# julienperriercornet/turbosqueeze

Measured on AMD Instinct MI355X. Metric: encode+decode GB/s on enwik9-shaped input (round trip of uncompressed bytes), higher is better.
Workload: dtype u8

## Files before the change

turbosqueeze_amd/csrc/tsq_dec_common.cuh:

```cuda
#pragma once

#include <type_traits>

#include "tsq_common.cuh"

namespace tsq {

#ifdef TSQ_STATS
__device__ unsigned long long g_dec_stats[16];
__device__ unsigned long long g_dec_wave[48];
#define TSQD_T0() unsigned long long t0_ = __builtin_amdgcn_s_memtime()
#define TSQD_ACC(slot) do { unsigned long long t1_ = __builtin_amdgcn_s_memtime(); st_[slot] += t1_ - t0_; t0_ = t1_; } while (0)
#define TSQD_CNT(slot, v) st_[slot] += (v)
#else
#define TSQD_T0() do {} while (0)
#define TSQD_ACC(slot) do {} while (0)
#define TSQD_CNT(slot, v) do {} while (0)
#endif

struct SymCfg {
    static constexpr uint32_t T = 1024;
    static constexpr uint32_t S = 6144;
    static constexpr uint32_t SPAD = 160;
    static constexpr uint32_t OUTC = 2 * S;
    static constexpr uint32_t HOP = 16;
    static constexpr uint32_t MAXG = 512;
    static constexpr uint32_t MAXSN = MAXG / HOP + 2;
    static constexpr uint32_t PER = S / T;
    static constexpr uint32_t TERM = S + SPAD;
    static constexpr uint32_t R = 65536 + OUTC + 64;
    static constexpr uint32_t RPAD = 64;
    static constexpr uint32_t SWORDS = (S + SPAD + 16) / 16;
};
static_assert(SymCfg::R % 16 == 0, "ring phase");
static_assert(SymCfg::R == 77888 && SymCfg::R % 64 == 0, "the record scan skews the ring by out_at & 63: the 64-position grid of the bit map falls on the ring's");
static_assert(SymCfg::OUTC == 12 * SymCfg::T, "twelve bytes per lane");
static_assert(SymCfg::S % SymCfg::T == 0 && SymCfg::SWORDS <= SymCfg::T, "lane counts");
static_assert(SymCfg::MAXG <= SymCfg::T / 2 && SymCfg::MAXG % SymCfg::HOP == 0 && SymCfg::MAXG >= SymCfg::S / 13 + 2 * SymCfg::HOP, "group table");
static_assert(4 * SymCfg::MAXG <= 2 * SymCfg::T, "at most two pairs per lane");

__device__ __forceinline__ void pair_lens(uint32_t sb, uint32_t cc, uint32_t ext, uint32_t& slen, uint32_t& olen)
{
    const uint32_t hi = sb >> 4, lo = sb & 15u;
    const uint32_t lit_hi = cc & 2u, lit_lo = cc & 1u;
    const uint32_t o_hi = (!lit_hi && ext && hi < 3u) ? (hi + 2u) << 4 : hi + 1u;
    const uint32_t o_lo = (!lit_lo && ext && lo < 3u) ? (lo + 2u) << 4 : lo + 1u;
    slen = 1u + (lit_hi ? hi + 1u : 2u) + (lit_lo ? lo + 1u : 2u);
    olen = o_hi + o_lo;
}

struct Image {
    uint32_t op, len, at;
    __device__ __forceinline__ uint32_t lead() const { return at & 3u; }
    __device__ __forceinline__ uint32_t a0() const { return at & ~3u; }
};

__device__ __forceinline__ uint4 prefetch_words(const uint8_t* in, uint32_t at, uint32_t av)
{
    using C = SymCfg;
    const uint32_t tid = threadIdx.x;
    const uint32_t lim = av < C::S + C::SPAD ? av : C::S + C::SPAD;
    uint4 w = make_uint4(0, 0, 0, 0);
    if (tid < C::SWORDS && (tid << 4) + 16u <= lim) __builtin_memcpy(&w, in + at + (tid << 4), 16);
    return w;
}
template <class L>
__device__ __forceinline__ void stage_words(uint8_t* lds, const uint8_t* in, uint32_t at, uint32_t av, uint4 pre)
{
    using C = SymCfg;
    const uint32_t tid = threadIdx.x;
    if (tid < C::SWORDS) {
        uint4 w = pre;
        const uint32_t lim = av < C::S + C::SPAD ? av : C::S + C::SPAD, o = tid << 4;
        if (o < lim && o + 16u > lim) {
            uint32_t b[4] = {0, 0, 0, 0};
            for (uint32_t k = 0; o + k < lim; ++k) b[k >> 2] |= (uint32_t)in[at + o + k] << (8u * (k & 3u));
            w = make_uint4(b[0], b[1], b[2], b[3]);
        }
        *reinterpret_cast<uint4*>(lds + L::sbuf + (tid << 4)) = w;
    }
}

template <class L>
__device__ __forceinline__ void parse_groups(uint8_t* lds, uint32_t slim, uint32_t (&x)[SymCfg::PER])
{
    using C = SymCfg;
    const uint32_t tid = threadIdx.x;
    const uint8_t* const sbuf = lds + L::sbuf;
    uint32_t y[C::PER], c[C::PER];
    {
        uint32_t* const pl = reinterpret_cast<uint32_t*>(lds + L::j4);
        constexpr uint32_t NW = (C::S + C::SPAD) / 4u;
#pragma unroll
        for (uint32_t k = 0; k < (NW + C::T - 1u) / C::T; ++k) {
            const uint32_t w = tid + k * C::T;
            if (w < NW) {
                const uint32_t v = reinterpret_cast<const uint32_t*>(sbuf)[w];
                uint32_t q[4];
#pragma unroll
                for (uint32_t b = 0; b < 4; ++b) {
                    const uint32_t hi = (v >> (8u * b + 4u)) & 15u, lo = (v >> (8u * b)) & 15u;
                    q[b] = 0x03040405u + (lo << 8) + (hi << 16) + ((lo + hi) << 24);
                }
                *reinterpret_cast<uint4*>(pl + 4u * w) = make_uint4(q[0], q[1], q[2], q[3]);
            }
        }
    }
    __syncthreads();
    {
        const uint32_t* const pl = reinterpret_cast<const uint32_t*>(lds + L::j4);
#pragma unroll
        for (uint32_t k = 0; k < C::PER; ++k) { const uint32_t o = tid + k * C::T; c[k] = (uint32_t)sbuf[o] << 3; x[k] = o + 1u; }
#pragma unroll
        for (uint32_t pr = 0; pr < 4; ++pr) {
#pragma unroll
            for (uint32_t k = 0; k < C::PER; ++k) y[k] = pl[x[k]];
#pragma unroll
            for (uint32_t k = 0; k < C::PER; ++k) x[k] += __builtin_amdgcn_ubfe(y[k], (c[k] >> (6u - 2u * pr)) & 0x18u, 8u);
        }
    }
    uint8_t* const j1 = lds + L::j1;
#pragma unroll
    for (uint32_t k = 0; k < C::PER; ++k) { const uint32_t o = tid + k * C::T; j1[o] = (uint8_t)(x[k] - o); x[k] = o < slim ? x[k] : C::TERM; }
    __syncthreads();
}

template <class L>
__device__ __forceinline__ void double_pointers(uint8_t* lds, uint32_t slim, uint32_t (&x)[SymCfg::PER])
{
    using C = SymCfg;
    const uint32_t tid = threadIdx.x;
    const uint8_t* const j1 = lds + L::j1;
    uint16_t* const j2 = reinterpret_cast<uint16_t*>(lds + L::j2);
    uint16_t* const j4 = reinterpret_cast<uint16_t*>(lds + L::j4);
    uint16_t* const j8 = reinterpret_cast<uint16_t*>(lds + L::j8);
    uint16_t* const j16 = reinterpret_cast<uint16_t*>(lds + L::j16);
    uint32_t y[C::PER];
#pragma unroll
    for (uint32_t k = 0; k < C::PER; ++k) { const uint32_t a = x[k] < slim ? x[k] : 0u; y[k] = a + j1[a]; }
#pragma unroll
    for (uint32_t k = 0; k < C::PER; ++k) { x[k] = x[k] < slim ? y[k] : C::TERM; j2[tid + k * C::T] = (uint16_t)x[k]; }
    if (tid <= C::SPAD) { j2[C::S + tid] = (uint16_t)C::TERM; j4[C::S + tid] = (uint16_t)C::TERM; j8[C::S + tid] = (uint16_t)C::TERM; j16[C::S + tid] = (uint16_t)C::TERM; }
    __syncthreads();
    const uint16_t* src = j2;
    uint16_t* const dsts[3] = {j4, j8, j16};
#pragma unroll
    for (uint32_t d = 0; d < 3; ++d) {
#pragma unroll
        for (uint32_t k = 0; k < C::PER; ++k) y[k] = src[x[k]];
#pragma unroll
        for (uint32_t k = 0; k < C::PER; ++k) { x[k] = y[k]; dsts[d][tid + k * C::T] = (uint16_t)x[k]; }
        __syncthreads();
        src = dsts[d];
    }
}

template <class L>
__device__ __forceinline__ uint32_t walk_chain(uint8_t* lds, uint32_t first, uint32_t slim)
{
    using C = SymCfg;
    const uint16_t* const j16 = reinterpret_cast<const uint16_t*>(lds + L::j16);
    uint16_t* const sn = reinterpret_cast<uint16_t*>(lds + L::sn);
    uint32_t* const misc = reinterpret_cast<uint32_t*>(lds + L::misc);
    if (threadIdx.x < 64u) {
        uint32_t x = first, k = 0;
        while (x < slim && k < C::MAXSN) {
            const uint32_t x1 = j16[x];
            const uint32_t x2 = j16[x1];
            sn[k++] = (uint16_t)x;
            if (x1 < slim && k < C::MAXSN) { sn[k++] = (uint16_t)x1; x = x2; }
            else x = x1;
        }
        if (threadIdx.x == 0) { misc[0] = k; if (k >= C::MAXSN && x < slim) misc[4] = kErrStream; }
    }
    __syncthreads();
    return misc[0];
}

template <class L>
__device__ __forceinline__ void group_lanes(uint8_t* lds, uint32_t nsn, uint32_t slim, uint32_t op, uint32_t size, uint32_t ext)
{
    using C = SymCfg;
    const uint32_t tid = threadIdx.x, lane = tid & 63u, wid = tid >> 6;
    const uint8_t* const sbuf = lds + L::sbuf;
    const uint8_t* const j1 = lds + L::j1;
    const uint16_t* const j2 = reinterpret_cast<const uint16_t*>(lds + L::j2);
    const uint16_t* const j4 = reinterpret_cast<const uint16_t*>(lds + L::j4);
    const uint16_t* const j8 = reinterpret_cast<const uint16_t*>(lds + L::j8);
    const uint16_t* const sn = reinterpret_cast<const uint16_t*>(lds + L::sn);
    uint16_t* const gstart = reinterpret_cast<uint16_t*>(lds + L::gstart);
    uint16_t* const glen = reinterpret_cast<uint16_t*>(lds + L::glen);
    uint32_t* const gout = reinterpret_cast<uint32_t*>(lds + L::gout);
    uint32_t* const pairs = reinterpret_cast<uint32_t*>(lds + L::pairs);
    uint32_t* const wsum = reinterpret_cast<uint32_t*>(lds + L::wsum);
    uint32_t* const misc = reinterpret_cast<uint32_t*>(lds + L::misc);
    uint32_t x = C::TERM;
    if (tid < nsn * C::HOP) {
        x = sn[tid >> 4];
        if (tid & 8u) x = j8[x];
        if (tid & 4u) x = j4[x];
        if (tid & 2u) x = j2[x];
        if (tid & 1u) x = x < slim ? (uint32_t)(x + j1[x]) : C::TERM;
    }
    uint32_t v = 0;
    if (x < slim) {
        gstart[tid] = (uint16_t)x;
        const uint32_t c = sbuf[x];
        uint32_t p = x + 1u, pw[4];
#pragma unroll
        for (uint32_t pr = 0; pr < 4; ++pr) {
            const uint32_t cc = (c >> (6u - 2u * pr)) & 3u;
            pw[pr] = p | (v << 13) | (cc << 30);
            uint32_t sl, ol;
            pair_lens(sbuf[p], cc, ext, sl, ol);
            p += sl;
            v += ol;
        }
        *reinterpret_cast<uint4*>(pairs + tid * 4u) = make_uint4(pw[0], pw[1], pw[2], pw[3]);
        glen[tid] = (uint16_t)v;
        if (p >= slim) { misc[1] = tid + 1u; misc[5] = p; }
    }
    const uint32_t incl = wave_scan_add(v);
    if (lane == 63) wsum[wid] = incl;
    __syncthreads();
    const uint32_t totals = wave_scan_add(lane < C::T / 64u ? wsum[lane] : 0u);
    const uint32_t before = wid ? (uint32_t)__builtin_amdgcn_readlane((int)totals, (int)wid - 1) : 0u;
    const uint32_t excl = before + incl - v;
    if (x < slim) {
        gout[tid] = op + excl;
        if (excl + 512u + 16u > C::OUTC) atomicMin(&misc[2], tid);
        if (op + excl + v >= size) atomicMin(&misc[3], tid);
    }
}

struct ChunkEnd {
    uint32_t ng;
    uint32_t next_at;
    uint32_t next_op;
    bool last;
    bool cut;
};
template <class L>
__device__ __forceinline__ ChunkEnd chunk_end(const uint8_t* lds, uint32_t op, uint32_t size)
{
    const uint16_t* const gstart = reinterpret_cast<const uint16_t*>(lds + L::gstart);
    const uint16_t* const glen = reinterpret_cast<const uint16_t*>(lds + L::glen);
    const uint32_t* const gout = reinterpret_cast<const uint32_t*>(lds + L::gout);
    const uint32_t* const misc = reinterpret_cast<const uint32_t*>(lds + L::misc);
    const uint32_t ng = misc[1], cut = misc[2], fin = misc[3];
    if (fin != 0xFFFFFFFFu && fin < cut) return {fin + 1u, 0u, size, true, false};
    if (cut != 0xFFFFFFFFu) return {cut, gstart[cut], gout[cut], false, true};
    return {ng, misc[5], ng ? gout[ng - 1] + glen[ng - 1] : op, false, false};
}

template <class L>
__device__ __forceinline__ void clear_records(uint8_t* lds)
{
    uint32_t* const recw = reinterpret_cast<uint32_t*>(lds + L::recw);
    for (uint32_t w = threadIdx.x; w < (SymCfg::OUTC + 16) / 4; w += SymCfg::T) *reinterpret_cast<uint4*>(recw + 4u * w) = make_uint4(0, 0, 0, 0);
}
template <class L, class PairAt>
__device__ __forceinline__ void drop_records(uint8_t* lds, uint32_t ng, const Image& im, uint32_t size, uint32_t avail, uint32_t ext,
                                             PairAt pair_at)
{
    using C = SymCfg;
    const uint32_t tid = threadIdx.x;
    const uint8_t* const sbuf = lds + L::sbuf;
    uint32_t* const recw = reinterpret_cast<uint32_t*>(lds + L::recw);
    const uint32_t op = im.op, lead = im.lead(), a0 = im.a0();
    if (tid == 0 && lead) recw[0] = 0x40000000u | (L::ring + a0);
    uint32_t bad = 0;
#pragma unroll
    for (uint32_t rep = 0; rep < 2; ++rep) {
        const uint32_t gi = tid + rep * C::T;
        if (gi >= ng * 4u) break;
        const uint2 pg = pair_at(rep, gi);
        const uint32_t pw = pg.x;
        uint32_t p = pw & 0x1FFFu, j = pg.y + ((pw >> 13) & 0x3FFFu);
        const uint32_t origin = j;
        uint32_t sb = 0;
        if (j < size) { if (p >= avail) bad = 1; sb = sbuf[p]; p++; }
#pragma unroll
        for (uint32_t sidx = 0; sidx < 2; ++sidx) {
            if (j < size && !bad) {
                const uint32_t nib = sidx == 0 ? sb >> 4 : sb & 15u;
                const uint32_t lit = (pw >> (31u - sidx)) & 1u;
                const uint32_t room = size - j;
                const uint32_t ij = j - op + lead;
                if (lit) {
                    const uint32_t len = nib + 1u, take = len < room ? len : room;
                    if (p + take > avail) bad = 1;
                    else recw[ij] = 0x40000000u | ((L::sbuf + p - ij) & 0xFFFFFFu);
                    p += len; j += take;
                } else {
                    if (p + 2u > avail) bad = 1;
                    const uint32_t off = (uint32_t)sbuf[p] | ((uint32_t)sbuf[p + 1] << 8);
                    p += 2;
                    const uint32_t len = ext ? nibble_span(nib) : nib + 1u;
                    const uint32_t take = len < room ? len : room;
                    if (off > origin || take > off) bad = 1;
                    if (!bad) {
                        const uint32_t a = origin - off;
                        const uint32_t n_hist = a >= op ? 0u : (op - a < take ? op - a : take);
                        if (n_hist) {
                            uint32_t x0 = a0 + C::R - ((op - a) - lead);
                            x0 -= x0 >= C::R ? C::R : 0u;
                            recw[ij] = 0x40000000u | ((L::ring + x0 - ij) & 0xFFFFFFu);
                            if (x0 + n_hist > C::R) { const uint32_t n1 = C::R - x0; recw[ij + n1] = 0x40000000u | ((L::ring - (ij + n1)) & 0xFFFFFFu); }
                        }
                        if (n_hist < take) recw[ij + n_hist] = 0xC0000000u | ((a - j) & 0xFFFFFFu);
                    }
                    j += take;
                }
            }
        }
    }
    if (bad) reinterpret_cast<uint32_t*>(lds + L::misc)[4] = kErrStream;
}

typedef __attribute__((address_space(3))) uint16_t lds_u16;

template <class L>
__device__ __forceinline__ uint32_t fetch_bytes(uint8_t* lds, const Image& im)
{
    const uint32_t tid = threadIdx.x, lane = tid & 63u, wid = tid >> 6;
    const uint32_t* const recw = reinterpret_cast<const uint32_t*>(lds + L::recw);
    uint32_t* const wsum = reinterpret_cast<uint32_t*>(lds + L::wsum);
    lds_u16* const wl = (lds_u16*)(lds + L::plist) + 768u * wid;
    const uint32_t own = 12u * tid;
    uint32_t r[12];
    {
        const uint4 q0 = *reinterpret_cast<const uint4*>(recw + own), q1 = *reinterpret_cast<const uint4*>(recw + own + 4u),
                    q2 = *reinterpret_cast<const uint4*>(recw + own + 8u);
        r[0] = q0.x; r[1] = q0.y; r[2] = q0.z; r[3] = q0.w; r[4] = q1.x; r[5] = q1.y; r[6] = q1.z; r[7] = q1.w; r[8] = q2.x; r[9] = q2.y; r[10] = q2.z; r[11] = q2.w;
#pragma unroll
        for (uint32_t k = 1; k < 12; ++k) r[k] = r[k] ? r[k] : r[k - 1];
        const uint32_t upto = wave_scan_last(r[11]);
        uint32_t carry = (uint32_t)__builtin_amdgcn_update_dpp(0, (int)upto, 0x138, 0xF, 0xF, false);
        if (lane == 63) wsum[wid] = upto;
        __syncthreads();
        {
            const uint32_t ws = lane < 16u ? wsum[lane] : 0u;
            const uint64_t m = __ballot(ws != 0u && lane < wid);
            const uint32_t prev = m ? (uint32_t)__builtin_amdgcn_readlane((int)ws, 63 - __builtin_clzll(m)) : 0u;
            carry = carry ? carry : prev;
        }
#pragma unroll
        for (uint32_t k = 0; k < 12; ++k) r[k] = r[k] ? r[k] : carry;
    }
    uint32_t pend = 0;
    if (own < im.lead() + im.len) {
        uint32_t v[12], by[12];
#pragma unroll
        for (uint32_t k = 0; k < 12; ++k) {
            v[k] = own + k + (uint32_t)((int32_t)(r[k] << 8) >> 8);
// ... 212 lines not shown
```

turbosqueeze_amd/csrc/tsq_dec_sym.cuh:

```cuda
#pragma once

#include "tsq_common.cuh"
#include "tsq_dec_common.cuh"

namespace tsq {

struct SymLds {
    static constexpr uint32_t sbuf = 0;
    static constexpr uint32_t j1 = sbuf + 16 * SymCfg::SWORDS;
    static constexpr uint32_t JN = (SymCfg::S + SymCfg::SPAD + 8u) & ~7u;
    static constexpr uint32_t j2 = j1 + SymCfg::S;
    static constexpr uint32_t j4 = j2 + 2 * JN;
    static constexpr uint32_t j8 = j4 + 2 * JN;
    static constexpr uint32_t j16 = j8 + 2 * JN;
    static constexpr uint32_t recw = j1;
    static constexpr uint32_t ent = j1;
    static constexpr uint32_t plist = ent + 2 * (SymCfg::OUTC + 16);
    static constexpr uint32_t gstart = j16 + 2 * JN;
    static constexpr uint32_t glen = gstart + 2 * SymCfg::MAXG;
    static constexpr uint32_t gout = glen + 2 * SymCfg::MAXG;
    static constexpr uint32_t pairs = gout + 4 * SymCfg::MAXG;
    static constexpr uint32_t sn = pairs + 16 * SymCfg::MAXG;
    static constexpr uint32_t wsum = (sn + 2 * ((SymCfg::MAXSN + 7) & ~7u) + 15) & ~15u;
    static constexpr uint32_t misc = wsum + 64;
    static constexpr uint32_t ring = (misc + 64 + 15) & ~15u;
    static constexpr uint32_t total = ring + SymCfg::R + SymCfg::RPAD;
    static_assert(recw % 16 == 0 && recw + 4 * (SymCfg::OUTC + 16) <= gstart && plist % 16 == 0 && plist + 2 * SymCfg::OUTC <= gstart,
                  "records, byte entries and waiting lists fit the dead doubling tables");
};
static_assert(SymLds::total <= 160 * 1024, "LDS budget");

struct RangeItem {
    uint32_t block, lo, hi, pad;
    uint64_t out_at;
};

struct BlockGroup {
    uint32_t block, first, count, hi;
};

enum DecMode : int { kDecWhole, kDecWindow, kDecGroup, kDecMark, kDecFind };

struct GroupCursor {
    uint32_t cur = 0, cur_lo = 0;
    uint32_t held = 0xFFFFFFFFu;
    RangeItem it = {0u, 0u, 0u, 0u, 0ull};
};

template <class L>
__device__ __forceinline__ void flush_group(const uint8_t* lds, uint8_t* out, const Image& im, const RangeItem* items, uint32_t count, GroupCursor& gc,
                                            uint32_t first_tid, uint32_t n_threads)
{
    using C = SymCfg;
    const uint32_t tid = threadIdx.x;
    if (im.len == 0 || tid < first_tid || gc.cur >= count || gc.cur_lo >= im.op + im.len) return;
    uint32_t& cur = gc.cur;
    const uint8_t* const ring = lds + L::ring;
    const uint32_t lane = tid & 63u, w = (tid - first_tid) >> 6, nw = n_threads >> 6;
    const uint32_t im_end = im.op + im.len;
    uint32_t pass0 = 0;
    bool leading = true;
    for (uint32_t base = cur & ~63u; base < count; base += 64u) {
        const uint32_t k = base + lane;
        RangeItem it = {0u, 0xFFFFFFFFu, 0u, 0u, 0ull};
        if (base == gc.held) it = gc.it;
        else if (k < count) it = items[k];
        const bool in_run = it.lo < im_end;
        if (leading) {
            gc.held = base; gc.it = it;
            const uint64_t done = __ballot(k < count && it.hi <= im.op);
            const uint32_t n = ~done == 0ull ? 64u : (uint32_t)__builtin_ctzll(~done);
            cur = base + n;
            leading = n == 64u;
            if (!leading) gc.cur_lo = (uint32_t)__builtin_amdgcn_readlane((int)it.lo, (int)n);
        }
        const uint32_t a = it.lo > im.op ? it.lo : im.op, b = it.hi < im_end ? it.hi : im_end;
        const bool live = in_run && a < b;
        const uint32_t len = live ? b - a : 0u;
        const uint64_t addr = (uint64_t)(uintptr_t)out + it.out_at + (a - it.lo);
        const uint32_t nwords = live ? (((uint32_t)addr & 15u) + len + 15u) >> 4 : 0u;
        uint32_t ra = im.at + (a - im.op); ra -= ra >= C::R ? C::R : 0u;
        uint32_t incl = nwords;
#pragma unroll
        for (uint32_t d = 1; d < 64u; d <<= 1) {
            const uint32_t up = __shfl_up(incl, d);
            if (lane >= d) incl += up;
        }
        const uint32_t total = (uint32_t)__builtin_amdgcn_readlane((int)incl, 63);
        const uint32_t passes = (total + 63u) >> 6;
        const uint32_t packed = len | (ra << 14);
        for (uint32_t j = (w + nw - pass0 % nw) % nw; j < passes; j += nw) {
            const uint32_t q = (j << 6) + lane;
            uint32_t t = 0;
#pragma unroll
            for (uint32_t step = 32u; step != 0u; step >>= 1) {
                const uint32_t v = __shfl(incl, (int)(t + step - 1u));
                t += v <= q ? step : 0u;
            }
            const bool act = q < total;
            const int src = (int)(t & 63u);
            const uint32_t excl_s = __shfl(incl - nwords, src), alo = __shfl((uint32_t)addr, src), ahi = __shfl((uint32_t)(addr >> 32), src),
                           pk = __shfl(packed, src);
            if (act) {
                const uint32_t kk = q - excl_s, slen = pk & 0x3FFFu, sra = pk >> 14, s = alo & 15u;
                uint8_t* const word = reinterpret_cast<uint8_t*>((uintptr_t)((((uint64_t)ahi << 32) | alo) & ~15ull)) + ((size_t)kk << 4);
                const int32_t i0 = (int32_t)(kk << 4) - (int32_t)s;
                const uint32_t e0 = kk == 0u ? s : 0u;
                const uint32_t left = (uint32_t)((int32_t)slen - i0), e1 = left < 16u ? left : 16u;
                int32_t r = (int32_t)sra + i0;
                r += r < 0 ? (int32_t)C::R : 0; r -= r >= (int32_t)C::R ? (int32_t)C::R : 0;
                const uint32_t r0 = (uint32_t)r & ~15u;
                uint32_t r1 = r0 + 16u; r1 -= r1 >= C::R ? C::R : 0u;
                const uint4 x = *reinterpret_cast<const uint4*>(ring + r0), y = *reinterpret_cast<const uint4*>(ring + r1);
                const uint32_t v8[8] = {x.x, x.y, x.z, x.w, y.x, y.y, y.z, y.w};
                const uint32_t dsh = ((uint32_t)r >> 2) & 3u, bsh = ((uint32_t)r & 3u) << 3;
                uint32_t u[5], o[4];
#pragma unroll
                for (uint32_t i = 0; i < 5u; ++i) u[i] = dsh == 0u ? v8[i] : dsh == 1u ? v8[i + 1] : dsh == 2u ? v8[i + 2] : v8[i + 3];
#pragma unroll
                for (uint32_t i = 0; i < 4u; ++i) o[i] = (uint32_t)((((uint64_t)u[i + 1] << 32) | u[i]) >> bsh);
                if (e0 == 0u && e1 == 16u) {
                    *reinterpret_cast<uint4*>(word) = make_uint4(o[0], o[1], o[2], o[3]);
                } else {
#pragma unroll
                    for (uint32_t i = 0; i < 4u; ++i) {
                        if (e0 <= 4u * i && 4u * i + 4u <= e1) {
                            *reinterpret_cast<uint32_t*>(word + 4u * i) = o[i];
                        } else {
#pragma unroll
                            for (uint32_t c = 0; c < 4u; ++c)
                                if (4u * i + c >= e0 && 4u * i + c < e1) word[4u * i + c] = (uint8_t)(o[i] >> (8u * c));
                        }
                    }
                }
            }
        }
        pass0 += passes;
        if (__ballot(!in_run) != 0ull) break;
    }
}

template <DecMode kMode>
__device__ __forceinline__ void sym_decode_block(const uint8_t* container, const FrameInfo* frames, uint32_t n_frames, const RangeItem* items,
                                                 uint8_t* outbuf, int32_t* status, const BlockGroup* groups = nullptr, uint32_t n_items = 0u,
                                                 [[maybe_unused]] uint32_t delim = 0u, [[maybe_unused]] uint64_t map_words = 0ull,
                                                 [[maybe_unused]] FindNeedle needle = {0ull, 0ull, 0u}, [[maybe_unused]] uint8_t* edges = nullptr)
{
    constexpr bool kWindow = kMode == kDecWindow, kGroup = kMode == kDecGroup, kMark = kMode == kDecMark, kFind = kMode == kDecFind;
    using C = SymCfg;
    using L = SymLds;
    extern __shared__ __attribute__((aligned(16))) uint8_t lds[];
    const uint32_t* const gout = reinterpret_cast<const uint32_t*>(lds + L::gout);
    const uint32_t* const pairs = reinterpret_cast<const uint32_t*>(lds + L::pairs);
    uint32_t* const misc = reinterpret_cast<uint32_t*>(lds + L::misc);

    const uint32_t tid = threadIdx.x;
    if (tid == 0) misc[11] = (uint32_t)*status;
    __syncthreads();
    if (misc[11] != 0u) return;
    uint32_t blk = blockIdx.x, lo = 0, hi = 0;
    uint64_t out_at = 0;
    if constexpr (kWindow) {
        const RangeItem it = items[blockIdx.x];
        if (it.block >= n_frames) {
            if (tid == 0) atomicMax(status, kErrStream);
            return;
        }
        blk = it.block; lo = it.lo; hi = it.hi; out_at = it.out_at;
    }
    [[maybe_unused]] const RangeItem* gitems = nullptr;
    [[maybe_unused]] uint32_t gcount = 0;
    [[maybe_unused]] GroupCursor gcur;
    if constexpr (kGroup) {
        const BlockGroup g = groups[blockIdx.x];
        if (g.block >= n_frames || g.count == 0u || g.first > n_items || g.count > n_items - g.first) {
            if (tid == 0) atomicMax(status, kErrStream);
            return;
        }
        blk = g.block; hi = g.hi; gitems = items + g.first; gcount = g.count;
    }
    const FrameInfo f = frames[blk];
    if (f.stream_len < 3u || f.stream_len > kSlotSize || f.out_len > kBlockSize || ((kWindow || kGroup) && (lo >= hi || hi > f.out_len))) {
        if (tid == 0) atomicMax(status, kErrStream);
        return;
    }
    const uint8_t* const in = container + f.stream_at;
    uint8_t* const out = kGroup || kMark || kFind ? outbuf : outbuf + (kWindow ? out_at : f.out_at);
    const uint32_t in_len = f.stream_len, size = f.out_len, ext = f.ext;
    const uint32_t oskew = kMark || kFind ? (uint32_t)(f.out_at & 63u) : kGroup ? 0u : (uint32_t)(((uintptr_t)out - lo) & 15u);

#ifdef TSQ_STATS
    const uint32_t lane = tid & 63u, wid = tid >> 6;
    unsigned long long st_[16] = {0};
    unsigned long long wj_[3] = {0, 0, 0};
#endif
    TSQD_T0();
    if (tid == 0) { misc[4] = 0; misc[9] = 0; misc[10] = 0; }
    uint32_t sp = 3, op = 0;
    uint32_t ring_op = oskew;
    Image prev = {0, 0, 0};
    uint4 pre = prefetch_words(in, sp, in_len - sp);
    bool staged_ahead = false;
    __syncthreads();

    while (op < size) {
        const uint32_t avail = in_len - sp;
        const uint32_t slim = avail < C::S ? avail : C::S;
        if (!staged_ahead) stage_words<L>(lds, in, sp, avail, pre);
        if (tid == 0) { misc[0] = 0; misc[1] = 0; misc[2] = 0xFFFFFFFFu; misc[3] = 0xFFFFFFFFu; misc[5] = 0; }
        __syncthreads();
        TSQD_ACC(0); TSQD_CNT(12, 1);

        uint32_t x[C::PER];
        parse_groups<L>(lds, slim, x);
        TSQD_ACC(1);
        double_pointers<L>(lds, slim, x);
        TSQD_ACC(2);
        const uint32_t nsn = walk_chain<L>(lds, 0u, slim);
        TSQD_ACC(3);

        if (tid >= C::T / 2) {
            if constexpr (kFind) flush_find<L>(lds, reinterpret_cast<uint32_t*>(out), map_words, f.out_at, blk, prev, needle, size, edges, C::T / 2, C::T / 2);
            else if constexpr (kMark) flush_mark<L>(lds, reinterpret_cast<uint32_t*>(out), map_words, f.out_at, blk, prev, delim, C::T / 2, C::T / 2);
            else if constexpr (kGroup) flush_group<L>(lds, out, prev, gitems, gcount, gcur, C::T / 2, C::T / 2);
            else if constexpr (kWindow) flush_window<L>(lds, out, prev, lo, hi, C::T / 2, C::T / 2);
            else flush_image<L>(lds, out, prev, C::T / 2, C::T / 2);
        }
        group_lanes<L>(lds, nsn, slim, op, size, ext);
        clear_records<L>(lds);
        __syncthreads();
        const ChunkEnd e = chunk_end<L>(lds, op, size);
        const uint32_t next_sp = sp + e.next_at;
        if (misc[4] != 0 || e.ng == 0 || (!e.last && next_sp >= in_len)) {
            if (tid == 0) atomicMax(status, kErrStream);
            return;
        }
        const Image im = {op, e.next_op - op, ring_op};
        const bool more = !e.last && !((kWindow || kGroup) && e.next_op >= hi);
        if (more) pre = prefetch_words(in, next_sp, in_len - next_sp);
        TSQD_ACC(4);

        drop_records<L>(lds, e.ng, im, size, avail, ext,
                        [&](uint32_t, uint32_t gi) { return make_uint2(pairs[gi], gout[gi >> 2]); });
        __syncthreads();
        if (misc[4] != 0) { if (tid == 0) atomicMax(status, (int32_t)misc[4]); return; }
        TSQD_ACC(5);
        const uint32_t n_wait = fetch_bytes<L>(lds, im);
        __syncthreads();
        TSQD_ACC(6);
        if (more) { stage_words<L>(lds, in, next_sp, in_len - next_sp, pre); staged_ahead = true; }
#ifdef TSQ_STATS
        const unsigned long long wj0_ = __builtin_amdgcn_s_memtime();
#endif
        [[maybe_unused]] const uint32_t iters = jump_pointers<L>(lds, n_wait);
#ifdef TSQ_STATS
        if (lane == 0) { atomicMax(&misc[9], iters); atomicAdd(&misc[10], n_wait); }
        if (lane == 0 && blockIdx.x == 0) { wj_[0] += __builtin_amdgcn_s_memtime() - wj0_; wj_[1] += n_wait; wj_[2] += iters; }
#endif
        __syncthreads();
        write_ring<L>(lds, im);
        TSQD_ACC(7);
#ifdef TSQ_STATS
        if (tid == 0) { st_[14] += misc[9]; st_[11] += misc[10]; misc[9] = 0; misc[10] = 0; }
#endif

        prev = im;
        ring_op += im.len; ring_op -= ring_op >= C::R ? C::R : 0u;
        op = e.next_op;
        sp = next_sp;
        TSQD_ACC(8);
        if (!more) break;
    }
    if constexpr (kGroup) { if (tid == C::T / 2) misc[12] = gcur.cur; }
    __syncthreads();
    if constexpr (kGroup) { if (tid < C::T / 2) gcur.cur = misc[12]; }
    if constexpr (kFind) flush_find<L>(lds, reinterpret_cast<uint32_t*>(out), map_words, f.out_at, blk, prev, needle, size, edges, 0, C::T);
    else if constexpr (kMark) flush_mark<L>(lds, reinterpret_cast<uint32_t*>(out), map_words, f.out_at, blk, prev, delim, 0, C::T);
    else if constexpr (kGroup) flush_group<L>(lds, out, prev, gitems, gcount, gcur, 0, C::T);
    else if constexpr (kWindow) flush_window<L>(lds, out, prev, lo, hi, 0, C::T);
    else flush_image<L>(lds, out, prev, 0, C::T);
#ifdef TSQ_STATS
    if (blockIdx.x == 0 && tid == 0) for (int q = 0; q < 16; ++q) g_dec_stats[q] = st_[q];
    if (blockIdx.x == 0 && lane == 0) for (int q = 0; q < 3; ++q) g_dec_wave[wid * 3 + q] = wj_[q];
#endif
}

__global__ __launch_bounds__(1024) void dec_sym_kernel(const uint8_t* __restrict__ container, const FrameInfo* __restrict__ frames,
                                                       uint8_t* __restrict__ outbuf, int32_t* __restrict__ status)
{
    sym_decode_block<kDecWhole>(container, frames, 0u, nullptr, outbuf, status);
}

__global__ __launch_bounds__(1024) void dec_item_kernel(const uint8_t* __restrict__ container, const FrameInfo* __restrict__ frames,
                                                        const uint32_t* __restrict__ owner, uint8_t* __restrict__ outbuf,
                                                        int32_t* __restrict__ item_status, const uint32_t* __restrict__ live_blocks)
{
    if (live_blocks && blockIdx.x >= *live_blocks) return;
    sym_decode_block<kDecWhole>(container, frames, 0u, nullptr, outbuf, item_status + owner[blockIdx.x]);
}

__global__ __launch_bounds__(1024) void dec_range_kernel(const uint8_t* __restrict__ container, const FrameInfo* __restrict__ frames, uint32_t n_frames,
                                                         const RangeItem* __restrict__ items, uint8_t* __restrict__ outbuf, int32_t* __restrict__ status)
{
    sym_decode_block<kDecWindow>(container, frames, n_frames, items, outbuf, status);
}

__global__ __launch_bounds__(1024) void dec_group_kernel(const uint8_t* __restrict__ container, const FrameInfo* __restrict__ frames, uint32_t n_frames,
                                                         const RangeItem* __restrict__ items, uint32_t n_items, const BlockGroup* __restrict__ groups,
                                                         uint8_t* __restrict__ outbuf, int32_t* __restrict__ status)
{
    sym_decode_block<kDecGroup>(container, frames, n_frames, items, outbuf, status, groups, n_items);
}

__global__ __launch_bounds__(1024) void dec_mark_kernel(const uint8_t* __restrict__ container, const FrameInfo* __restrict__ frames,
                                                        const int32_t* __restrict__ verdict, uint32_t delim, uint64_t* __restrict__ map,
                                                        uint64_t map_words, int32_t* __restrict__ status)
{
    if (verdict && *verdict != 0) return;
    sym_decode_block<kDecMark>(container, frames, 0u, nullptr, reinterpret_cast<uint8_t*>(map), status, nullptr, 0u, delim, map_words);
}

__global__ __launch_bounds__(1024) void dec_find_kernel(const uint8_t* __restrict__ container, const FrameInfo* __restrict__ frames,
                                                        const int32_t* __restrict__ verdict, uint32_t n0, uint32_t n1, uint32_t n2, uint32_t n3,
                                                        uint32_t m, uint64_t* __restrict__ map, uint64_t map_words, uint8_t* __restrict__ edges,
                                                        int32_t* __restrict__ status)
{
    if (verdict && *verdict != 0) return;
    const FindNeedle needle = {((uint64_t)n1 << 32) | n0, ((uint64_t)n3 << 32) | n2, m};
    sym_decode_block<kDecFind>(container, frames, 0u, nullptr, reinterpret_cast<uint8_t*>(map), status, nullptr, 0u, 0u, map_words, needle, edges);
}

}
```

turbosqueeze_amd/csrc/tsq_experiment.h:

```cpp
#pragma once

#if defined(TSQ_X_NOHAZ) || defined(TSQ_X_NOCOMMITWAIT) || defined(TSQ_X_NOPATCH) || defined(TSQ_X_FAKE_TABLE) || defined(TSQ_X_FAKE_CAND) || \
    defined(TSQ_X_FREE_QUERY)
#define TSQ_TIMING_ONLY_BUILD 1
#ifndef TSQ_EXPERIMENT
#error "a timing-only switch (TSQ_X_*: wrong streams on purpose) needs -DTSQ_EXPERIMENT; the product library is never built with one (tools/xbuild.sh)"
#endif
#else
#define TSQ_TIMING_ONLY_BUILD 0
#endif

#if defined(TSQ_STATS) || defined(TSQ_SPINS) || defined(TSQ_TRACEONLY) || defined(TSQ_REGION) || defined(TSQ_JITTER) || defined(TSQ_X_DELAY_STAGE)
#define TSQ_INSTRUMENTED_BUILD 1
#else
#define TSQ_INSTRUMENTED_BUILD 0
#endif
```

turbosqueeze_amd/csrc/tsq_runtime.hip:

```cpp
#include "tsq_internal.h"

#include "tsq_batch.cuh"
#include "tsq_common.cuh"
#include "tsq_container.cuh"
#include "tsq_format.h"
#include "tsq_serial.cuh"
#include "tsq_split.cuh"
#include "tsq_index.cuh"
#include "tsq_index_packed.cuh"
#include "tsq_join.cuh"
#include "tsq_cut.cuh"
#include "tsq_launch.cuh"
#include "tsq_gather.cuh"
#include "tsq_gather_sort.h"
#include "tsq_rows.cuh"
#include "tsq_records.cuh"
#include "tsq_find.cuh"

#include <algorithm>
#include <cstdarg>
#include <cstdio>
#include <cstring>
#include <memory>
#include <new>

using namespace tsq;

#define TSQ_HIP(ctx, call)                                                                       \
    do {                                                                                         \
        hipError_t e_ = (call);                                                                  \
        if (e_ != hipSuccess) {                                                                  \
            (ctx)->set_error("%s failed: %s", #call, hipGetErrorString(e_));                     \
            return TSQA_ERR_HIP;                                                                 \
        }                                                                                        \
    } while (0)

void tsqa_ctx::set_error(const char* fmt, ...)
{
    va_list ap;
    va_start(ap, fmt);
    vsnprintf(err, sizeof(err), fmt, ap);
    va_end(ap);
}

static hipStream_t stream_of(const tsqa_ctx* c, void* hip_stream) { return hip_stream ? static_cast<hipStream_t>(hip_stream) : c->stream; }

extern "C" size_t tsqa_block_count(size_t n) { return (n + kBlockSize - 1) / kBlockSize; }

extern "C" size_t tsqa_container_bound(size_t n) { return 16 + tsqa_block_count(n) * (size_t)(3 + kSlotSize); }

#define TSQ_STR2(x) #x
#define TSQ_STR(x) TSQ_STR2(x)
#if !defined(TSQ_LM) || !defined(TSQ_LF) || !defined(TSQ_RECORDS)
#error "tsqa_build_info stringifies TSQ_LM, TSQ_LF and TSQ_RECORDS: tsq_enc_stage.cuh (through tsq_launch.cuh) goes above it"
#endif
extern "C" const char* tsqa_build_info(void)
{
    return "arch=gfx950 timing_only=" TSQ_STR(TSQ_TIMING_ONLY_BUILD) " instrumented=" TSQ_STR(TSQ_INSTRUMENTED_BUILD)
#ifdef TSQ_AB_VARIANTS
           " ab_variants=1"
#else
           " ab_variants=0"
#endif
           " lm=" TSQ_STR(TSQ_LM) " lf=" TSQ_STR(TSQ_LF) " records=" TSQ_STR(TSQ_RECORDS) " [switches:"
#ifdef TSQ_X_NOHAZ
           " TSQ_X_NOHAZ"
#endif
#ifdef TSQ_X_NOCOMMITWAIT
           " TSQ_X_NOCOMMITWAIT"
#endif
#ifdef TSQ_X_NOPATCH
           " TSQ_X_NOPATCH"
#endif
#ifdef TSQ_X_FAKE_TABLE
           " TSQ_X_FAKE_TABLE"
#endif
#ifdef TSQ_X_FAKE_CAND
           " TSQ_X_FAKE_CAND"
#endif
#ifdef TSQ_X_FREE_QUERY
           " TSQ_X_FREE_QUERY"
#endif
#ifdef TSQ_X_DELAY_STAGE
           " TSQ_X_DELAY_STAGE"
#endif
#ifdef TSQ_STATS
           " TSQ_STATS"
#endif
#ifdef TSQ_SPINS
           " TSQ_SPINS"
#endif
#ifdef TSQ_TRACEONLY
           " TSQ_TRACEONLY"
#endif
#ifdef TSQ_JITTER
           " TSQ_JITTER"
#endif
#if !TSQ_TIMING_ONLY_BUILD && !TSQ_INSTRUMENTED_BUILD
           " none"
#endif
           "]";
}

extern "C" int tsqa_create(int device, tsqa_ctx** out)
{
    if (!out) return TSQA_ERR_ARG;
    *out = nullptr;
    int count = 0;
    if (hipGetDeviceCount(&count) != hipSuccess || count <= 0) return TSQA_ERR_NO_DEVICE;
    if (device < 0) { if (hipGetDevice(&device) != hipSuccess) return TSQA_ERR_NO_DEVICE; }
    if (device >= count) return TSQA_ERR_ARG;
    hipDeviceProp_t prop;
    if (hipGetDeviceProperties(&prop, device) != hipSuccess) return TSQA_ERR_NO_DEVICE;
    if (strncmp(prop.gcnArchName, "gfx950", 6) != 0) {
        fprintf(stderr, "turbosqueeze_amd: device %d is %s; this library carries gfx950 code only\n", device, prop.gcnArchName);
        return TSQA_ERR_NO_DEVICE;
    }
    tsqa_ctx* c = new (std::nothrow) tsqa_ctx();
    if (!c) return TSQA_ERR_ARG;
    c->device = device;
    c->n_cus = prop.multiProcessorCount;
    if (const char* e = getenv("TSQ_AMD_DECODE_WAIT_LIMIT")) { const long v = atol(e); if (v > 0) c->decode_wait_limit = (uint32_t)v; }
    if (hipSetDevice(device) != hipSuccess || hipStreamCreateWithFlags(&c->stream, hipStreamNonBlocking) != hipSuccess) {
        delete c;
        return TSQA_ERR_HIP;
    }
    if (!c->d_size.grow(c, 1) || !c->d_status.grow(c, 1)) {
        tsqa_destroy(c);
        return TSQA_ERR_HIP;
    }
    *out = c;
    return TSQA_OK;
}

extern "C" void tsqa_destroy(tsqa_ctx* c)
{
    if (!c) return;
    (void)hipSetDevice(c->device);
    if (c->stream) { (void)hipStreamSynchronize(c->stream); (void)hipStreamDestroy(c->stream); }
    for (hipEvent_t e : c->prof_pool) if (e) (void)hipEventDestroy(e);
    if (c->host_frames_copied) (void)hipEventDestroy(c->host_frames_copied);
    c->range_up.destroy(); c->batch_up.destroy();
    delete c;
}

extern "C" const char* tsqa_last_error(const tsqa_ctx* c) { return c ? c->err : "null context"; }
extern "C" int tsqa_device_id(const tsqa_ctx* c) { return c ? c->device : -1; }
extern "C" void tsqa_set_kernel_variant(tsqa_ctx* c, int ev, int dv) { if (c) { c->enc_variant = ev; c->dec_variant = dv; } }
extern "C" void tsqa_set_decode_wait_limit(tsqa_ctx* c, uint32_t polls) { if (c) c->decode_wait_limit = polls ? polls : 1u; }

int tsqa_ctx::reserve(size_t n_blocks, bool want_tables, bool want_slots, bool all_streams, hipStream_t s)
{
    (void)hipSetDevice(device);
    const size_t nb = n_blocks, n_at = nb ? nb + 1 : 0;
    const size_t n_slots = want_slots && nb ? nb * (size_t)kSlotSize + 256 : 0, n_tables = want_tables ? nb * (size_t)kHashEntries : 0;
    const bool descriptors = sizes.needs(nb) || frame_at.needs(n_at) || frames.needs(nb) || block_owner.needs(nb);
    if (!descriptors && !slots.needs(n_slots) && !tables.needs(n_tables)) return TSQA_OK;
    if (all_streams) (void)hipDeviceSynchronize(); else wait_for(s);
    if (descriptors) forget_sharded();
    return sizes.grow(this, nb) && frame_at.grow(this, n_at) && frames.grow(this, nb) && block_owner.grow(this, nb) &&
           slots.grow(this, n_slots) && tables.grow(this, n_tables) ? TSQA_OK : TSQA_ERR_HIP;
}

int tsqa_ctx::reserve_duo(size_t n_blocks, hipStream_t s)
{
    (void)hipSetDevice(device);
    const size_t n_ring = n_blocks * (size_t)DuoCfg::SLOTS * DuoCfg::REC_WORDS, n_flags = n_blocks * (size_t)DuoCfg::FLAG_STRIDE;
    if (!duo_ring.needs(n_ring) && !duo_flags.needs(n_flags)) return TSQA_OK;
    wait_for(s);
    return duo_ring.grow(this, n_ring) && duo_flags.grow(this, n_flags) ? TSQA_OK : TSQA_ERR_HIP;
}

static size_t doubled(size_t from, size_t n)
{
    if (n == 0) return 0;
    while (from < n) from *= 2;
    return from;
}

int tsqa_ctx::reserve_host_frames(size_t n)
{
    (void)hipSetDevice(device);
    if (host_frames_pending) { (void)hipEventSynchronize(host_frames_copied); host_frames_pending = false; }
    if (!host_frames_copied) TSQ_HIP(this, hipEventCreateWithFlags(&host_frames_copied, hipEventDisableTiming));
    if (host_frames.needs(n)) TSQ_HIP(this, host_frames.grow(doubled(64, n)));
    host_frame_src.resize(host_frames.cap);
    return TSQA_OK;
}

int tsqa_uploads::acquire(tsqa_ctx* c, size_t bytes, Slot* slot)
{
    (void)hipSetDevice(c->device);
    const int k = next_;
    next_ ^= 1;
    if (pending_[k]) { (void)hipEventSynchronize(done_[k]); pending_[k] = false; }
    if (!done_[k]) TSQ_HIP(c, hipEventCreateWithFlags(&done_[k], hipEventDisableTiming));
    if (dev_[k].needs(bytes)) {
        const size_t want = doubled(4096, bytes);
        host_[k].reset(); dev_[k].reset();
        TSQ_HIP(c, host_[k].grow(want));
        if (!dev_[k].grow(c, want)) return TSQA_ERR_HIP;
    }
    *slot = Slot{this, k};
    return TSQA_OK;
}

void tsqa_uploads::destroy()
{
    for (int k = 0; k < 2; ++k)
        if (done_[k]) (void)hipEventDestroy(done_[k]);
}

int tsqa_ctx::reserve_batch(size_t n_items)
{
    (void)hipSetDevice(device);
    const size_t want = doubled(256, n_items), one = want ? 1 : 0;
    if (!batch_at.needs(want) && !batch_sizes.needs(want) && !batch_offsets.needs(want + one) && !batch_heads.needs(want * kHeaderSize) &&
        !batch_status.needs(want) && !batch_items.needs(want) && !batch_live.needs(one)) return TSQA_OK;
    (void)hipDeviceSynchronize();
    return batch_at.grow(this, want) && batch_sizes.grow(this, want) && batch_offsets.grow(this, want + one) &&
           batch_heads.grow(this, want * kHeaderSize) && batch_status.grow(this, want) && batch_items.grow(this, want) &&
           batch_live.grow(this, one) ? TSQA_OK : TSQA_ERR_HIP;
}

int tsqa_ctx::reserve_tables(size_t n_blocks, size_t n_launches, bool want_items)
{
    (void)hipSetDevice(device);
    const size_t blocks = doubled(256, n_blocks), launches = doubled(16, n_launches), owners = want_items ? blocks : 0;
    if (!table_blocks.needs(blocks) && !table_launch_item.needs(launches) && !table_block_item.needs(owners)) return TSQA_OK;
    (void)hipDeviceSynchronize();
    return table_blocks.grow(this, blocks) && table_launch_item.grow(this, launches) && table_block_item.grow(this, owners) ? TSQA_OK : TSQA_ERR_HIP;
}

int tsqa_ctx::reserve_join(size_t n_items)
// ... 2750 lines not shown
```

Measured before the change: 22.77.

## Build pointer-jumping with two doubling tables instead of four in symbol decoder

The decoder's pointer doubling now stores only a 4-hop and a 16-hop table. It reaches the 4-hop table by walking the 1-hop byte table three times in registers, and the 16-hop table by chaining the 4-hop table three times. This cuts two LDS table writes and two block barriers. The group lane seeding then uses up to three 4-hop plus three 1-hop lookups instead of one lookup per power of two, trading more dependent LDS reads for fewer syncs and less LDS. The group tables move down over the freed space, and a timing-only experimental switch is added that skips parsing by replaying cached tables.

```diff
diff --git a/turbosqueeze_amd/csrc/tsq_dec_common.cuh b/turbosqueeze_amd/csrc/tsq_dec_common.cuh
--- a/turbosqueeze_amd/csrc/tsq_dec_common.cuh
+++ b/turbosqueeze_amd/csrc/tsq_dec_common.cuh
@@ -131,28 +131,30 @@
     using C = SymCfg;
     const uint32_t tid = threadIdx.x;
     const uint8_t* const j1 = lds + L::j1;
-    uint16_t* const j2 = reinterpret_cast<uint16_t*>(lds + L::j2);
     uint16_t* const j4 = reinterpret_cast<uint16_t*>(lds + L::j4);
-    uint16_t* const j8 = reinterpret_cast<uint16_t*>(lds + L::j8);
     uint16_t* const j16 = reinterpret_cast<uint16_t*>(lds + L::j16);
     uint32_t y[C::PER];
 #pragma unroll
-    for (uint32_t k = 0; k < C::PER; ++k) { const uint32_t a = x[k] < slim ? x[k] : 0u; y[k] = a + j1[a]; }
-#pragma unroll
-    for (uint32_t k = 0; k < C::PER; ++k) { x[k] = x[k] < slim ? y[k] : C::TERM; j2[tid + k * C::T] = (uint16_t)x[k]; }
-    if (tid <= C::SPAD) { j2[C::S + tid] = (uint16_t)C::TERM; j4[C::S + tid] = (uint16_t)C::TERM; j8[C::S + tid] = (uint16_t)C::TERM; j16[C::S + tid] = (uint16_t)C::TERM; }
+    for (uint32_t h = 0; h < 3; ++h) {
+#pragma unroll
+        for (uint32_t k = 0; k < C::PER; ++k) { const uint32_t a = x[k] < slim ? x[k] : 0u; y[k] = a + j1[a]; }
+#pragma unroll
+        for (uint32_t k = 0; k < C::PER; ++k) x[k] = x[k] < slim ? y[k] : C::TERM;
+    }
+#pragma unroll
+    for (uint32_t k = 0; k < C::PER; ++k) j4[tid + k * C::T] = (uint16_t)x[k];
+    if (tid <= C::SPAD) { j4[C::S + tid] = (uint16_t)C::TERM; j16[C::S + tid] = (uint16_t)C::TERM; }
     __syncthreads();
-    const uint16_t* src = j2;
-    uint16_t* const dsts[3] = {j4, j8, j16};
-#pragma unroll
-    for (uint32_t d = 0; d < 3; ++d) {
-#pragma unroll
-        for (uint32_t k = 0; k < C::PER; ++k) y[k] = src[x[k]];
-#pragma unroll
-        for (uint32_t k = 0; k < C::PER; ++k) { x[k] = y[k]; dsts[d][tid + k * C::T] = (uint16_t)x[k]; }
-        __syncthreads();
-        src = dsts[d];
-    }
+#pragma unroll
+    for (uint32_t h = 0; h < 3; ++h) {
+#pragma unroll
+        for (uint32_t k = 0; k < C::PER; ++k) y[k] = j4[x[k]];
+#pragma unroll
+        for (uint32_t k = 0; k < C::PER; ++k) x[k] = y[k];
+    }
+#pragma unroll
+    for (uint32_t k = 0; k < C::PER; ++k) j16[tid + k * C::T] = (uint16_t)x[k];
+    __syncthreads();
 }
 
 template <class L>
@@ -184,9 +186,7 @@
     const uint32_t tid = threadIdx.x, lane = tid & 63u, wid = tid >> 6;
     const uint8_t* const sbuf = lds + L::sbuf;
     const uint8_t* const j1 = lds + L::j1;
-    const uint16_t* const j2 = reinterpret_cast<const uint16_t*>(lds + L::j2);
     const uint16_t* const j4 = reinterpret_cast<const uint16_t*>(lds + L::j4);
-    const uint16_t* const j8 = reinterpret_cast<const uint16_t*>(lds + L::j8);
     const uint16_t* const sn = reinterpret_cast<const uint16_t*>(lds + L::sn);
     uint16_t* const gstart = reinterpret_cast<uint16_t*>(lds + L::gstart);
     uint16_t* const glen = reinterpret_cast<uint16_t*>(lds + L::glen);
@@ -197,10 +197,11 @@
     uint32_t x = C::TERM;
     if (tid < nsn * C::HOP) {
         x = sn[tid >> 4];
-        if (tid & 8u) x = j8[x];
-        if (tid & 4u) x = j4[x];
-        if (tid & 2u) x = j2[x];
-        if (tid & 1u) x = x < slim ? (uint32_t)(x + j1[x]) : C::TERM;
+        const uint32_t h4 = (tid >> 2) & 3u, h1 = tid & 3u;
+#pragma unroll
+        for (uint32_t h = 0; h < 3; ++h) if (h < h4) x = j4[x];
+#pragma unroll
+        for (uint32_t h = 0; h < 3; ++h) if (h < h1) x = x < slim ? (uint32_t)(x + j1[x]) : C::TERM;
     }
     uint32_t v = 0;
     if (x < slim) {
diff --git a/turbosqueeze_amd/csrc/tsq_dec_sym.cuh b/turbosqueeze_amd/csrc/tsq_dec_sym.cuh
--- a/turbosqueeze_amd/csrc/tsq_dec_sym.cuh
+++ b/turbosqueeze_amd/csrc/tsq_dec_sym.cuh
@@ -9,14 +9,12 @@
     static constexpr uint32_t sbuf = 0;
     static constexpr uint32_t j1 = sbuf + 16 * SymCfg::SWORDS;
     static constexpr uint32_t JN = (SymCfg::S + SymCfg::SPAD + 8u) & ~7u;
-    static constexpr uint32_t j2 = j1 + SymCfg::S;
-    static constexpr uint32_t j4 = j2 + 2 * JN;
-    static constexpr uint32_t j8 = j4 + 2 * JN;
-    static constexpr uint32_t j16 = j8 + 2 * JN;
+    static constexpr uint32_t j4 = j1 + SymCfg::S;
+    static constexpr uint32_t j16 = j4 + 2 * JN;
     static constexpr uint32_t recw = j1;
     static constexpr uint32_t ent = j1;
     static constexpr uint32_t plist = ent + 2 * (SymCfg::OUTC + 16);
-    static constexpr uint32_t gstart = j16 + 2 * JN;
+    static constexpr uint32_t gstart = recw + 4 * (SymCfg::OUTC + 16);
     static constexpr uint32_t glen = gstart + 2 * SymCfg::MAXG;
     static constexpr uint32_t gout = glen + 2 * SymCfg::MAXG;
     static constexpr uint32_t pairs = gout + 4 * SymCfg::MAXG;
@@ -26,9 +24,14 @@
     static constexpr uint32_t ring = (misc + 64 + 15) & ~15u;
     static constexpr uint32_t total = ring + SymCfg::R + SymCfg::RPAD;
     static_assert(recw % 16 == 0 && recw + 4 * (SymCfg::OUTC + 16) <= gstart && plist % 16 == 0 && plist + 2 * SymCfg::OUTC <= gstart,
-                  "records, byte entries and waiting lists fit the dead doubling tables");
+                  "records, byte entries and waiting lists lie over the dead doubling tables, below the group tables");
+    static_assert(j4 % 16 == 0 && j4 + 4 * (SymCfg::S + SymCfg::SPAD) <= gstart && j16 + 2 * JN <= gstart, "P1's pair lengths and both doubling tables");
 };
 static_assert(SymLds::total <= 160 * 1024, "LDS budget");
+#ifdef TSQ_X_DEC_FREEPARSE
+struct SymLdsX { static constexpr uint32_t sbuf = SymLds::pairs; };
+static_assert(SymLdsX::sbuf % 16 == 0 && 16 * SymCfg::SWORDS <= 16 * SymCfg::MAXG, "the stream fits the pair words");
+#endif
 
 struct RangeItem {
     uint32_t block, lo, hi, pad;
@@ -201,21 +204,40 @@
     Image prev = {0, 0, 0};
     uint4 pre = prefetch_words(in, sp, in_len - sp);
     bool staged_ahead = false;
+#ifdef TSQ_X_DEC_FREEPARSE
+    constexpr uint32_t kXWarm = 8;
+    constexpr uint32_t kXTab = (L::j16 + 2 * L::JN - L::j1) / 16;
+    static_assert((L::j16 + 2 * L::JN - L::j1) % 16 == 0 && kXTab <= 2 * C::T, "two words per lane");
+    uint4 xtab[2] = {make_uint4(0, 0, 0, 0), make_uint4(0, 0, 0, 0)};
+    uint32_t xsp = sp;
+    uint32_t xn = 0;
+#endif
     __syncthreads();
 
     while (op < size) {
         const uint32_t avail = in_len - sp;
         const uint32_t slim = avail < C::S ? avail : C::S;
         if (!staged_ahead) stage_words<L>(lds, in, sp, avail, pre);
+#ifdef TSQ_X_DEC_FREEPARSE
+        if (xn > kXWarm) for (uint32_t q = 0; q < 2; ++q) if (tid + q * C::T < kXTab) *reinterpret_cast<uint4*>(lds + L::j1 + 16u * (tid + q * C::T)) = xtab[q];
+#endif
         if (tid == 0) { misc[0] = 0; misc[1] = 0; misc[2] = 0xFFFFFFFFu; misc[3] = 0xFFFFFFFFu; misc[5] = 0; }
         __syncthreads();
         TSQD_ACC(0); TSQD_CNT(12, 1);
 
         uint32_t x[C::PER];
+#ifdef TSQ_X_DEC_FREEPARSE
+        if (xn <= kXWarm) {
+            parse_groups<L>(lds, slim, x);
+            double_pointers<L>(lds, slim, x);
+            if (xn == kXWarm) for (uint32_t q = 0; q < 2; ++q) if (tid + q * C::T < kXTab) xtab[q] = *reinterpret_cast<const uint4*>(lds + L::j1 + 16u * (tid + q * C::T));
+        }
+#else
         parse_groups<L>(lds, slim, x);
         TSQD_ACC(1);
         double_pointers<L>(lds, slim, x);
         TSQD_ACC(2);
+#endif
         const uint32_t nsn = walk_chain<L>(lds, 0u, slim);
         TSQD_ACC(3);
 
@@ -237,7 +259,12 @@
         }
         const Image im = {op, e.next_op - op, ring_op};
         const bool more = !e.last && !((kWindow || kGroup) && e.next_op >= hi);
+#ifdef TSQ_X_DEC_FREEPARSE
+        xsp = xsp + e.next_at < in_len ? xsp + e.next_at : 3u;
+        if (more) pre = prefetch_words(in, xsp, in_len - xsp);
+#else
         if (more) pre = prefetch_words(in, next_sp, in_len - next_sp);
+#endif
         TSQD_ACC(4);
 
         drop_records<L>(lds, e.ng, im, size, avail, ext,
@@ -248,7 +275,11 @@
         const uint32_t n_wait = fetch_bytes<L>(lds, im);
         __syncthreads();
         TSQD_ACC(6);
+#ifdef TSQ_X_DEC_FREEPARSE
+        if (more) { if (xn < kXWarm) stage_words<L>(lds, in, xsp, in_len - xsp, pre); else stage_words<SymLdsX>(lds, in, xsp, in_len - xsp, pre); staged_ahead = true; }
+#else
         if (more) { stage_words<L>(lds, in, next_sp, in_len - next_sp, pre); staged_ahead = true; }
+#endif
 #ifdef TSQ_STATS
         const unsigned long long wj0_ = __builtin_amdgcn_s_memtime();
 #endif
@@ -267,6 +298,9 @@
         prev = im;
         ring_op += im.len; ring_op -= ring_op >= C::R ? C::R : 0u;
         op = e.next_op;
+#ifdef TSQ_X_DEC_FREEPARSE
+        if (xn++ < kXWarm)
+#endif
         sp = next_sp;
         TSQD_ACC(8);
         if (!more) break;
diff --git a/turbosqueeze_amd/csrc/tsq_experiment.h b/turbosqueeze_amd/csrc/tsq_experiment.h
--- a/turbosqueeze_amd/csrc/tsq_experiment.h
+++ b/turbosqueeze_amd/csrc/tsq_experiment.h
@@ -1,7 +1,7 @@
 #pragma once
 
 #if defined(TSQ_X_NOHAZ) || defined(TSQ_X_NOCOMMITWAIT) || defined(TSQ_X_NOPATCH) || defined(TSQ_X_FAKE_TABLE) || defined(TSQ_X_FAKE_CAND) || \
-    defined(TSQ_X_FREE_QUERY)
+    defined(TSQ_X_FREE_QUERY) || defined(TSQ_X_DEC_FREEPARSE)
 #define TSQ_TIMING_ONLY_BUILD 1
 #ifndef TSQ_EXPERIMENT
 #error "a timing-only switch (TSQ_X_*: wrong streams on purpose) needs -DTSQ_EXPERIMENT; the product library is never built with one (tools/xbuild.sh)"
diff --git a/turbosqueeze_amd/csrc/tsq_runtime.hip b/turbosqueeze_amd/csrc/tsq_runtime.hip
--- a/turbosqueeze_amd/csrc/tsq_runtime.hip
+++ b/turbosqueeze_amd/csrc/tsq_runtime.hip
@@ -80,6 +80,9 @@
 #endif
 #ifdef TSQ_X_FREE_QUERY
            " TSQ_X_FREE_QUERY"
+#endif
+#ifdef TSQ_X_DEC_FREEPARSE
+           " TSQ_X_DEC_FREEPARSE"
 #endif
 #ifdef TSQ_X_DELAY_STAGE
            " TSQ_X_DELAY_STAGE"
```

Measured after the change: 22.75, median of 2. Within noise of the previous version (-0.1%).
